# gmarcais/Jellyfish

Hardware: NVIDIA H100
Metric: k-mers counted/sec at k=21 (higher is better)
Workload: dtype u64

## Files before the change

jellyfish_b200/csrc/jf_device.cuh:

```cuda
#ifndef JF_DEVICE_CUH
#define JF_DEVICE_CUH
#include <stdint.h>
#include <cuda_runtime.h>
#include <type_traits>

namespace jfk {

constexpr int HALO  = 256;
constexpr int PRE   = 64;

enum { ST_H = 0, ST_S = 1, ST_L = 2 };
constexpr uint32_t SYM_BREAK = 4;

enum { STAT_KMERS = 0, STAT_INSERTED, STAT_DISTINCT, STAT_REPROBES, STAT_OVERFLOWED,
       STAT_FAILED, STAT_FAIL_DROPPED, STAT_OVF_FULL, STAT_ROUTE_DROPPED, STAT_MAXCOUNT, STAT_POOL_FULL, STAT_FORMAT_ERR, STAT_N };

struct Carry {
  uint32_t state;
  uint32_t pad;
  uint8_t  sym[PRE];
};

struct TableDev {
  void*     slots;
  uint64_t  local_mask;
  uint32_t  local_lsize;
  uint32_t  lsize;
  uint32_t  shard_index;
  uint32_t  kbits;
  uint32_t  rbits;
  uint32_t  fbits;
  uint32_t  max_reprobe;
  uint32_t  op;
  unsigned long long* ovf_keys;
  unsigned long long* ovf_vals;
  uint64_t  ovf_mask;
  unsigned long long* stats;
  uint64_t* fail_keys;
  uint64_t* fail_counts;
  uint64_t  fail_cap;
};

enum { BLOOM_NONE = 0, BLOOM_FILTER = 1, BLOOM_COUNT = 2, BLOOM_CHECK = 3 };
struct BloomDev {
  uint32_t mode;
  uint32_t k;
  uint64_t m;
  uint64_t inv;
  uint32_t* bits;
  uint32_t* locks;
  uint32_t lock_mask;
  uint32_t pad;
  const uint64_t* lut1;
  const uint64_t* lut2;
};

struct u128 { uint64_t lo, hi; };

__host__ __device__ __forceinline__ uint64_t tri(uint32_t i) { return (uint64_t)i * (i + 1) / 2; }

__device__ __forceinline__ uint32_t smem_u32(const void* p) { return (uint32_t)__cvta_generic_to_shared(p); }

__device__ __forceinline__ void mbar_init(uint64_t* bar, uint32_t count) {
  asm volatile("mbarrier.init.shared::cta.b64 [%0], %1;" :: "r"(smem_u32(bar)), "r"(count) : "memory");
}
__device__ __forceinline__ void mbar_expect_tx(uint64_t* bar, uint32_t bytes) {
  asm volatile("mbarrier.arrive.expect_tx.shared::cta.b64 _, [%0], %1;" :: "r"(smem_u32(bar)), "r"(bytes) : "memory");
}
__device__ __forceinline__ void mbar_arrive(uint64_t* bar) {
  asm volatile("mbarrier.arrive.shared::cta.b64 _, [%0];" :: "r"(smem_u32(bar)) : "memory");
}
__device__ __forceinline__ bool mbar_try_wait(uint64_t* bar, uint32_t parity) {
  uint32_t ok;
  asm volatile("{\n\t.reg .pred p;\n\t"
               "mbarrier.try_wait.parity.shared::cta.b64 p, [%1], %2;\n\t"
               "selp.u32 %0, 1, 0, p;\n\t}"
               : "=r"(ok) : "r"(smem_u32(bar)), "r"(parity) : "memory");
  return ok != 0;
}
__device__ __forceinline__ void mbar_wait(uint64_t* bar, uint32_t parity) {
  while(!mbar_try_wait(bar, parity)) { }
}
__device__ __forceinline__ void tma_load_1d(void* dst, const void* src, uint32_t bytes, uint64_t* bar) {
  asm volatile("cp.async.bulk.shared::cluster.global.mbarrier::complete_tx::bytes [%0], [%1], %2, [%3];"
               :: "r"(smem_u32(dst)), "l"(src), "r"(bytes), "r"(smem_u32(bar)) : "memory");
}
__device__ __forceinline__ void tma_store_1d(void* dst, const void* src, uint32_t bytes) {
  asm volatile("cp.async.bulk.global.shared::cta.bulk_group [%0], [%1], %2;" :: "l"(dst), "r"(smem_u32(src)), "r"(bytes) : "memory");
}
__device__ __forceinline__ void tma_commit_group() { asm volatile("cp.async.bulk.commit_group;" ::: "memory"); }
__device__ __forceinline__ void tma_wait_group_read0() { asm volatile("cp.async.bulk.wait_group.read 0;" ::: "memory"); }
__device__ __forceinline__ void tma_wait_group0() { asm volatile("cp.async.bulk.wait_group 0;" ::: "memory"); }
__device__ __forceinline__ void fence_proxy_async() {
  asm volatile("fence.proxy.async.shared::cta;" ::: "memory");
}

__device__ __forceinline__ u128 atomic_cas_128(void* addr, u128 cmp, u128 val) {
  u128 old;
  asm volatile("{\n\t.reg .b128 c, s, d;\n\t"
               "mov.b128 c, {%2, %3};\n\t"
               "mov.b128 s, {%4, %5};\n\t"
               "atom.global.relaxed.gpu.cas.b128 d, [%6], c, s;\n\t"
               "mov.b128 {%0, %1}, d;\n\t}"
               : "=l"(old.lo), "=l"(old.hi)
               : "l"(cmp.lo), "l"(cmp.hi), "l"(val.lo), "l"(val.hi), "l"(addr) : "memory");
  return old;
}
__device__ __forceinline__ u128 load_128(const void* addr) {
  u128 v;
  asm volatile("ld.global.relaxed.gpu.v2.u64 {%0, %1}, [%2];" : "=l"(v.lo), "=l"(v.hi) : "l"(addr) : "memory");
  return v;
}

__host__ __device__ __forceinline__ uint32_t base_symbol(uint32_t b) {
  uint32_t u = b & 0xDFu;
  uint32_t x = (b >> 1) & 3u;
  uint32_t code = x ^ (x >> 1);
  bool ok = (u == 'A') | (u == 'C') | (u == 'G') | (u == 'T');
  return ok ? code : SYM_BREAK;
}
// ... 349 lines not shown
```

jellyfish_b200/csrc/jf_engine.cu:

```cuda
#include <cuda_runtime.h>
#include <algorithm>
#include <atomic>
#include <cmath>
#include <cstdio>
#include <cstring>
#include <string>
#include <vector>

#include "../../include/jfgpu.h"
#include "host/jf_matrix.hpp"
#include "jf_kernels.cuh"
#include "jf_extract.cuh"
#include "jf_window.cuh"
#include "jf_dump.cuh"
#include "jf_shard.cuh"

using namespace jfk;

static std::atomic<unsigned long long> g_launches(0);
static thread_local std::string g_create_error;

#define JF_LAUNCHED() g_launches.fetch_add(1, std::memory_order_relaxed)

namespace {
// ... 1042 lines not shown
  TableDev T = table_dev(e, e->tab);
  const uint64_t ns = e->tab.local_size + e->tab.margin;
  const int grid = (int)std::min<uint64_t>((ns + 255) / 256, (uint64_t)e->n_sm * 16);
  switch(e->tab.slot_bits) {
  case 32:  max_count_kernel<32><<<grid, 256, 0, e->cs>>>(T, ns); break;
  case 64:  max_count_kernel<64><<<grid, 256, 0, e->cs>>>(T, ns); break;
  default:  max_count_kernel<128><<<grid, 256, 0, e->cs>>>(T, ns); break;
  }
  JF_LAUNCHED();
  int rc = read_stats(e);
  if(rc) return rc;
  const uint64_t maxc = e->h_stats[STAT_MAXCOUNT];
  if(e->eff_val_len < 64 && (maxc >> e->eff_val_len) != 0) {
    e->eff_val_len = bitsize(maxc);
    if(!e->tab.M.is_identity()) {
      rc = rebuild_table(e, e->tab.lsize, jfb::gf2_matrix::identity(kbits), 0, 0);
      if(rc) return rc;
    }
  }
  return JFGPU_OK;
}

void resolve_kernel_events(jfgpu_engine* e) {
  for(size_t i = 0; i + 1 < e->kev_used; i += 2) {
    float ms = 0;
    if(cudaEventElapsedTime(&ms, e->kev[i], e->kev[i + 1]) == cudaSuccess) { e->kernel_ms += ms; e->kernel_launches++; }
    else cudaGetLastError();
  }
  e->kev_used = 0;
}

int check_after_batches(jfgpu_engine* e) {
  int rc = read_stats(e);
  if(rc) return rc;
  if(e->h_stats[STAT_OVF_FULL]) return fail(e, JFGPU_ERR_FULL, "counter overflow side table is full");
  if(e->h_stats[STAT_FAILED]) {
    if(e->part.pending) {
      rc = part_drain(e, e->cs);
      if(rc) return rc;
      rc = read_stats(e);
      if(rc) return rc;
      if(!e->h_stats[STAT_FAILED]) return JFGPU_OK;
    }
    return regrow(e);
  }
  return JFGPU_OK;
}

}

extern "C" {

const char* jfgpu_version(void) { return "jellyfish-b200 0.1 (sm_90a)"; }
uint64_t jfgpu_kernel_launches(void) { return g_launches.load(); }
const char* jfgpu_last_error(jfgpu_handle h) { return h ? h->err.c_str() : g_create_error.c_str(); }

void* jfgpu_host_alloc(size_t bytes) { void* p = nullptr; if(cudaHostAlloc(&p, bytes, cudaHostAllocDefault) != cudaSuccess) { cudaGetLastError(); return nullptr; } return p; }
void jfgpu_host_free(void* p) { if(p) cudaFreeHost(p); }
int jfgpu_memcpy_h2d(void* dev_dst, const void* host_src, size_t bytes, void* stream) {
  if(cudaMemcpyAsync(dev_dst, host_src, bytes, cudaMemcpyHostToDevice, (cudaStream_t)stream) != cudaSuccess) { cudaGetLastError(); return JFGPU_ERR_CUDA; }
  return JFGPU_OK;
}

int jfgpu_reference_matrix(uint32_t r, uint32_t c, uint32_t skip, uint64_t* cols) {
  if(r == 0 || r > 64 || c == 0 || !cols) return JFGPU_ERR_ARG;
  jfb::glibc_random rng;
  jfb::gf2_matrix res;
  for(uint32_t i = 0; i <= skip; ++i) { jfb::gf2_matrix m(r, c); res = m.randomize_pseudo_inverse(rng); }
  for(uint32_t i = 0; i < c; ++i) cols[i] = res[i];
  return JFGPU_OK;
}

int jfgpu_create(const jfgpu_params* params, jfgpu_handle* out) {
  if(!params || !out) return fail(nullptr, JFGPU_ERR_ARG, "null argument");
  if(params->struct_size != sizeof(jfgpu_params)) return fail(nullptr, JFGPU_ERR_ARG, "jfgpu_params size mismatch");
  if(params->k < 1 || params->k > 64) return fail(nullptr, JFGPU_ERR_ARG, "mer length must be in [1, 64]");
  if(params->size == 0) return fail(nullptr, JFGPU_ERR_ARG, "size must be positive");
  uint32_t ns = params->n_shards ? params->n_shards : 1;
  if(ns & (ns - 1)) return fail(nullptr, JFGPU_ERR_ARG, "n_shards must be a power of two");
  if(params->shard_index >= ns) return fail(nullptr, JFGPU_ERR_ARG, "shard_index out of range");
  if(params->max_reprobe > 255) return fail(nullptr, JFGPU_ERR_ARG, "max_reprobe must be <= 255");

  int ndev = 0;
  if(cudaGetDeviceCount(&ndev) != cudaSuccess || ndev == 0) {
    cudaGetLastError();
    return fail(nullptr, JFGPU_ERR_CUDA, "no CUDA device: the jellyfish-b200 engine has no CPU fallback");
  }
  if(params->device < 0 || params->device >= ndev) return fail(nullptr, JFGPU_ERR_ARG, "invalid device ordinal");

  jfgpu_engine* e = new jfgpu_engine;
  e->p = *params;
  e->p.n_shards = ns;
  e->device = params->device;
  e->k = params->k;
  e->kw = params->k > 32 ? 2 : 1;
  e->nbytes = (2 * params->k + 7) / 8;
  e->eff_val_len = params->counter_len;
  e->shard_bits = ceil_log2(ns);
  auto bail = [&](int code) { g_create_error = e->err; jfgpu_destroy(e); return code; };

  cudaError_t c;
  if((c = cudaSetDevice(e->device)) != cudaSuccess) { e->err = cudaGetErrorString(c); return bail(JFGPU_ERR_CUDA); }
  cudaDeviceProp prop;
  if((c = cudaGetDeviceProperties(&prop, e->device)) != cudaSuccess) { e->err = cudaGetErrorString(c); return bail(JFGPU_ERR_CUDA); }
  if(prop.major != 9 || prop.minor != 0) { e->err = "this engine is built for sm_90a (Hopper) only"; return bail(JFGPU_ERR_CUDA); }
  e->n_sm = prop.multiProcessorCount;
  if(cudaStreamCreateWithFlags(&e->cs, cudaStreamNonBlocking) != cudaSuccess ||
// ... 739 lines not shown
```

jellyfish_b200/csrc/jf_window.cuh:

```cuda
#pragma once

namespace jfk {

constexpr uint32_t WIN_TILE_UNITS = 4;
constexpr uint32_t WIN_MAX_G = 64;
constexpr uint32_t WIN_MAX_WPR = 2048;
constexpr uint32_t WIN_NTH = 512;

struct WinDev {
  uint32_t g0, G, wpr_lg, n_tiles;
  const uint32_t* lazy_win;
  uint32_t tile_first[WIN_MAX_G + 1];
  uint32_t stile_first[WIN_MAX_G + 1];
  uint32_t unit_first[WIN_MAX_G + 1];
  uint32_t* wstart;
  uint32_t* wcursor;
  uint32_t* wcnt;
  uint32_t* wrec; uint64_t wrec_cap;
  uint64_t* def_pos; uint32_t* def_high; unsigned long long* def_n; uint64_t def_cap;
};

__device__ __forceinline__ uint32_t win_region_of_tile(const WinDev& wd, uint32_t tile) {
  uint32_t r = 0;
  while(r + 1 < wd.G && wd.tile_first[r + 1] <= tile) ++r;
  return r;
}

__device__ __forceinline__ uint64_t win_slot_base(const WinDev& wd, uint32_t region_bits, uint32_t task) {
  return ((uint64_t)(wd.g0 + (task >> wd.wpr_lg)) << region_bits) + ((uint64_t)(task & ((1u << wd.wpr_lg) - 1)) << WIN_LG);
}

__global__ void __launch_bounds__(WIN_NTH) win_hist_kernel(PartDev pd, WinDev wd, const uint32_t* __restrict__ order, uint32_t hb) {
  __shared__ uint32_t cnt[WIN_MAX_WPR];
  const uint32_t wpr = 1u << wd.wpr_lg;
  for(uint32_t i = threadIdx.x; i < wpr; i += WIN_NTH) cnt[i] = 0;
  __syncthreads();
  const uint32_t r = win_region_of_tile(wd, blockIdx.x);
  const uint32_t u0 = wd.unit_first[r] + (blockIdx.x - wd.tile_first[r]) * WIN_TILE_UNITS;
  const uint32_t u1 = min(u0 + WIN_TILE_UNITS, wd.unit_first[r + 1]);
  uint32_t chunk[WIN_TILE_UNITS], n[WIN_TILE_UNITS]; uint4 v[WIN_TILE_UNITS];
#pragma unroll
  for(uint32_t j = 0; j < WIN_TILE_UNITS; ++j) chunk[j] = u0 + j < u1 ? __ldg(order + u0 + j) : 0u;
#pragma unroll
  for(uint32_t j = 0; j < WIN_TILE_UNITS; ++j) n[j] = u0 + j < u1 ? __ldg(&pd.dir[chunk[j]].y) : 0u;
#pragma unroll
  for(uint32_t j = 0; j < WIN_TILE_UNITS; ++j) {
    v[j] = make_uint4(0, 0, 0, 0);
    if(threadIdx.x * 4 < n[j]) v[j] = __ldg(reinterpret_cast<const uint4*>(pd.pool + (size_t)chunk[j] * CHUNK_BYTES) + threadIdx.x);
  }
#pragma unroll
  for(uint32_t j = 0; j < WIN_TILE_UNITS; ++j) {
    const uint32_t i = threadIdx.x * 4;
    const uint32_t rec[4] = { v[j].x, v[j].y, v[j].z, v[j].w };
// ... 56 lines not shown
  const uint32_t half = tid >> 9, piece = tid & 511u;
  const uint32_t wmask = wpr - 1;
#pragma unroll
  for(uint32_t it = 0; it < WIN_ST_UNITS / 2; ++it) {
    const uint32_t j = 2 * it + half, n = s_n[j];
    if(piece * 4 < n) {
      const uint4 v = __ldg(reinterpret_cast<const uint4*>(pd.pool + (size_t)s_chunk[j] * CHUNK_BYTES) + piece);
      const uint32_t rec[4] = { v.x, v.y, v.z, v.w };
#pragma unroll
      for(uint32_t q = 0; q < 4; ++q) if(piece * 4 + q < n) atomicAdd(&cnt[((rec[q] >> hb) >> WIN_LG) & wmask], 1u);
    }
  }
  __syncthreads();
  const uint32_t per = (wpr + WIN_ST_NTH - 1) / WIN_ST_NTH;
  const uint32_t b = tid * per;
  uint32_t s = 0;
  for(uint32_t i = b; i < min(b + per, wpr); ++i) s += cnt[i];
  uint32_t incl = s;
#pragma unroll
  for(int o = 1; o < 32; o <<= 1) { const uint32_t v = __shfl_up_sync(0xffffffffu, incl, o); if((tid & 31) >= (uint32_t)o) incl += v; }
  if((tid & 31) == 31) warp_tot[tid >> 5] = incl;
  __syncthreads();
  uint32_t woff = 0, total = 0;
  for(uint32_t w = 0; w < WIN_ST_NTH / 32; ++w) { const uint32_t x = warp_tot[w]; if(w < (tid >> 5)) woff += x; total += x; }
  uint32_t run = woff + incl - s;
  for(uint32_t i = b; i < min(b + per, wpr); ++i) {
    const uint32_t c = cnt[i];
    lbase[i] = run; lcur[i] = run;
    gbase[i] = (c ? atomicAdd(&wd.wcursor[(r << wd.wpr_lg) + i], c) : 0u) - run;
    run += c;
  }
  __syncthreads();
#pragma unroll
  for(uint32_t it = 0; it < WIN_ST_UNITS / 2; ++it) {
    const uint32_t j = 2 * it + half, n = s_n[j];
    if(piece * 4 < n) {
      const uint4 v = __ldcs(reinterpret_cast<const uint4*>(pd.pool + (size_t)s_chunk[j] * CHUNK_BYTES) + piece);
      const uint32_t rec[4] = { v.x, v.y, v.z, v.w };
#pragma unroll
      for(uint32_t q = 0; q < 4; ++q) if(piece * 4 + q < n) stage[atomicAdd(&lcur[((rec[q] >> hb) >> WIN_LG) & wmask], 1u)] = rec[q];
    }
  }
  __syncthreads();
  for(uint32_t i = tid; i < total; i += WIN_ST_NTH) {
    const uint32_t v = stage[i], w = ((v >> hb) >> WIN_LG) & wmask;
    const uint32_t dst = gbase[w] + i;
    if(dst < wd.wrec_cap) wd.wrec[dst] = v;
  }
}

constexpr uint32_t WIN2_NTH = 1024;
constexpr uint32_t WIN2_CONS = WIN2_NTH - 32;
constexpr uint32_t WIN2_RB  = 10240;
constexpr uint32_t WIN2_BLK = 256;
constexpr uint32_t WIN2_NONE = 0xFFFFFFFFu;
constexpr size_t   WIN2_SMEM = (size_t)2 * WIN_SLOTS * 4 + (size_t)2 * WIN2_RB * 4;

struct Win2Info { uint32_t task, b, n, pad; };

template<int KW>
__global__ void __launch_bounds__(WIN2_NTH, 1) win_insert2_kernel(TableDev T, PartDev pd, WinDev wd, const uint64_t* __restrict__ inv_lut_g, uint32_t nbytes) {
  extern __shared__ __align__(128) uint8_t w2smem[];
  __shared__ __align__(8) uint64_t full[2];
  __shared__ __align__(8) uint64_t empty[2];
  __shared__ Win2Info info[2];
  __shared__ uint32_t cursor[2];
  uint32_t* const winb0 = reinterpret_cast<uint32_t*>(w2smem);
  uint32_t* const recb0 = winb0 + 2 * WIN_SLOTS;
  uint32_t* tab = (uint32_t*)T.slots;
  const uint32_t n_tasks = wd.G << wd.wpr_lg;
  const uint32_t tid = threadIdx.x, lane = tid & 31u;

  auto slot_base_of = [&](uint32_t task) -> uint64_t { return win_slot_base(wd, pd.region_bits, task); };
  if(tid == 0) {
    mbar_init(&full[0], 1); mbar_init(&full[1], 1);
    mbar_init(&empty[0], WIN2_CONS / 32); mbar_init(&empty[1], WIN2_CONS / 32);
    fence_proxy_async();
  }
  __syncthreads();

  if(tid < 32) {
    const bool lead = lane == 0;
    uint32_t next_from = blockIdx.x;
    uint32_t ephase[2] = { 0, 0 };
    uint32_t cur_task[2] = { WIN2_NONE, WIN2_NONE }, cur_n[2] = { 0, 0 }, cur_b[2] = { 0, 0 };
    auto load_batch = [&](uint32_t s, uint32_t off, bool with_window) {
      const uint32_t nb = min(WIN2_RB, cur_n[s] - off);
      const uint32_t rbytes = ((nb + 3u) & ~3u) * 4u;
      cursor[s] = 0;
      mbar_expect_tx(&full[s], rbytes + (with_window ? WIN_SLOTS * 4u : 0u));
      if(with_window) tma_load_1d(winb0 + s * WIN_SLOTS, tab + slot_base_of(cur_task[s]), WIN_SLOTS * 4u, &full[s]);
      tma_load_1d(recb0 + s * WIN2_RB, wd.wrec + cur_b[s] + off, rbytes, &full[s]);
    };
    auto next_window = [&](uint32_t s) {
      uint32_t t = next_from, c = 0;
      while(t < n_tasks && (c = wd.wcnt[t]) == 0) t += gridDim.x;
      if(t >= n_tasks) {
        next_from = t; cur_task[s] = WIN2_NONE;
        if(lead) { info[s].task = WIN2_NONE; mbar_arrive(&full[s]); }
        return;
      }
      next_from = t + gridDim.x;
      cur_task[s] = t; cur_n[s] = c; cur_b[s] = wd.wstart[t];
      const bool fill = wd.lazy_win && wd.lazy_win[slot_base_of(t) >> WIN_LG] != WIN_IN_MEMORY;
      if(fill) {
        uint4* const w = reinterpret_cast<uint4*>(winb0 + s * WIN_SLOTS);
        for(uint32_t i = lane; i < WIN_SLOTS / 4; i += 32) w[i] = make_uint4(0, 0, 0, 0);
        fence_proxy_async();
        __syncwarp();
      }
      if(lead) {
        info[s].task = t; info[s].b = cur_b[s]; info[s].n = c;
        load_batch(s, 0, !fill);
      }
    };
    next_window(0); next_window(1);
    for(uint32_t s = 0; cur_task[s] != WIN2_NONE; s ^= 1u) {
      for(uint32_t off = WIN2_RB; off < cur_n[s]; off += WIN2_RB) {
        mbar_wait(&empty[s], ephase[s]); ephase[s] ^= 1u;
        if(lead) load_batch(s, off, false);
      }
      mbar_wait(&empty[s], ephase[s]); ephase[s] ^= 1u;
      if(lead) {
        tma_store_1d(tab + slot_base_of(cur_task[s]), winb0 + s * WIN_SLOTS, WIN_SLOTS * 4u);
        tma_commit_group();
        tma_wait_group_read0();
      }
      __syncwarp();
      next_window(s);
    }
    if(lead) tma_wait_group0();
    return;
  }

  const uint32_t fb = T.fbits, rb = T.rbits, hb = fb - rb;
  const uint32_t fmask = (1u << fb) - 1u, one = 1u << fb, cb = 32 - fb;
  const uint32_t hmask = hb ? ((1u << hb) - 1u) : 0u;
  const uint32_t lt_mask = (1u << lane) - 1u;
  uint32_t n_ins = 0, n_new = 0, n_rep = 0;
  uint32_t fphase[2] = { 0, 0 };
  for(uint32_t s = 0; ; s ^= 1u) {
    mbar_wait(&full[s], fphase[s]); fphase[s] ^= 1u;
    const Win2Info inf = info[s];
    if(inf.task == WIN2_NONE) break;
    uint32_t* const win = winb0 + s * WIN_SLOTS;
    const uint32_t* const recs = recb0 + s * WIN2_RB;
    const uint64_t slot_base = slot_base_of(inf.task);
    for(uint32_t off = 0; off < inf.n; off += WIN2_RB) {
      const uint32_t nb = min(WIN2_RB, inf.n - off);
      if(off) { mbar_wait(&full[s], fphase[s]); fphase[s] ^= 1u; }
      bool have = false, want = true;
      uint32_t rec = 0, local = 0, kf = 0, at = 0, p = 0;
      uint32_t blk_next = 0, blk_end = 0;
      bool more = true;
      for(;;) {
        const uint32_t need = __ballot_sync(0xffffffffu, want);
        if(need && more) {
          if(blk_next >= blk_end) {
            uint32_t base = 0;
            if(lane == 0) base = atomicAdd(&cursor[s], WIN2_BLK);
            blk_next = __shfl_sync(0xffffffffu, base, 0);
            blk_end = min(blk_next + WIN2_BLK, nb);
            more = blk_next < nb;
          }
          if(want && more) {
            const uint32_t i = blk_next + __popc(need & lt_mask);
            if(i < blk_end) {
              rec = recs[i];
              local = (rec >> hb) & (WIN_SLOTS - 1); kf = ((rec & hmask) << rb) | 1u;
              at = local; p = 0;
              have = true; want = false;
            }
          }
          blk_next = min(blk_next + (uint32_t)__popc(need), blk_end);
        }
        if(!__any_sync(0xffffffffu, have)) { if(!more) break; else continue; }
        if(have) {
          if(at < WIN_SLOTS) {
            const uint32_t o = atomicCAS(&win[at], 0u, kf | one);
            if(o == 0u) { ++n_new; ++n_ins; n_rep += p; want = true; }
            else if((o & fmask) == kf) {
              const uint32_t o2 = atomicAdd(&win[at], one);
              if((((o2 >> fb) + 1) >> cb) != 0) k2_carry(T.ovf_keys, T.ovf_vals, T.ovf_mask, T.stats, slot_base + at);
              ++n_ins; n_rep += p; want = true;
            } else if(p < T.max_reprobe) { ++p; at += p; ++kf; }
            else {
              k2_fail<KW>(T.shard_index, T.local_lsize, T.lsize, T.stats, T.fail_keys, T.fail_counts, T.fail_cap, slot_base + local, rec & hmask, inv_lut_g, nbytes);
              want = true;
            }
          } else {
            const unsigned long long d = atomicAdd(wd.def_n, 1ull);
            if(d < wd.def_cap) { wd.def_pos[d] = slot_base + local; wd.def_high[d] = rec & hmask; }
            else atomicAdd(&T.stats[STAT_POOL_FULL], 1ull);
            want = true;
          }
          have = !want;
        }
      }
      fence_proxy_async();
      __syncwarp();
      if(lane == 0) mbar_arrive(&empty[s]);
    }
  }
  unsigned long long v[3] = { n_ins, n_new, n_rep };
#pragma unroll
  for(int q = 0; q < 3; ++q) {
#pragma unroll
    for(int o = 16; o; o >>= 1) v[q] += __shfl_xor_sync(0xffffffffu, v[q], o);
  }
  if(lane == 0) {
    if(v[0]) atomicAdd(&T.stats[STAT_INSERTED], v[0]);
    if(v[1]) atomicAdd(&T.stats[STAT_DISTINCT], v[1]);
    if(v[2]) atomicAdd(&T.stats[STAT_REPROBES], v[2]);
  }
}

__global__ void __launch_bounds__(256) win_zero_kernel(uint32_t* __restrict__ tab, const uint32_t* __restrict__ state, const uint32_t* __restrict__ wcnt,
                                                       uint64_t w_first, uint32_t n) {
  const uint32_t lane = threadIdx.x & 31u;
  const uint32_t n_warps = gridDim.x * (blockDim.x / 32);
  for(uint32_t t = (blockIdx.x * blockDim.x + threadIdx.x) / 32; t < n; t += n_warps) {
    if((wcnt && wcnt[t]) || state[w_first + t] == WIN_IN_MEMORY) continue;
    uint4* const w = reinterpret_cast<uint4*>(tab + ((w_first + t) << WIN_LG));
    for(uint32_t i = lane; i < WIN_SLOTS / 4; i += 32) w[i] = make_uint4(0, 0, 0, 0);
  }
}

template<int KW>
__global__ void __launch_bounds__(256) win_deferred_kernel(TableDev T, WinDev wd, const uint64_t* __restrict__ inv_lut_g, uint32_t nbytes) {
  const uint32_t fb = T.fbits, rb = T.rbits;
  const uint32_t fmask = (1u << fb) - 1u, one = 1u << fb, cb = 32 - fb;
  uint32_t* tab = (uint32_t*)T.slots;
  const unsigned long long n = min(*wd.def_n, (unsigned long long)wd.def_cap);
  uint32_t n_ins = 0, n_new = 0, n_rep = 0;
  for(unsigned long long i = (unsigned long long)blockIdx.x * blockDim.x + threadIdx.x; i < n; i += (unsigned long long)gridDim.x * blockDim.x) {
    const uint64_t base = wd.def_pos[i];
    const uint32_t high = wd.def_high[i], kf0 = high << rb;
    bool ok = true;
    const uint32_t o = atomicCAS(&tab[base], 0u, (kf0 | 1u) | one);
    if(o == 0u) ++n_new;
    else if((o & fmask) == (kf0 | 1u)) {
      const uint32_t o2 = atomicAdd(&tab[base], one);
      if((((o2 >> fb) + 1) >> cb) != 0) k2_carry(T.ovf_keys, T.ovf_vals, T.ovf_mask, T.stats, base);
    } else {
      const uint32_t w = k2_walk(tab, base, kf0, fb, T.max_reprobe);
      ok = w != 0;
      if(ok) {
        const uint32_t p = (w & 0xFFFFu) - 1;
        n_rep += p; if(w & 0x10000u) ++n_new;
        if(w & 0x20000u) k2_carry(T.ovf_keys, T.ovf_vals, T.ovf_mask, T.stats, base + tri(p));
      }
    }
    if(ok) ++n_ins;
    else k2_fail<KW>(T.shard_index, T.local_lsize, T.lsize, T.stats, T.fail_keys, T.fail_counts, T.fail_cap, base, high, inv_lut_g, nbytes);
  }
  unsigned long long v[3] = { n_ins, n_new, n_rep };
// ... 14 lines not shown
```

Before: 36.20 billion.

## Restructure window insert pipeline: batched metadata lookup, early record prefetch, two-phase probing

The producer warp now scans window metadata 32 tasks at a time with a ballot, and issues the next window's record TMA load before waiting on the store of the current window, so the loads overlap the write-back. Consumer warps now do a vectorized first-probe pass over 64-record blocks, two records per lane. Records that collide go into a per-warp shared-memory queue and are reprobed in a second phase, which keeps lanes busy and lets the kernel use smaller blocks. It also adds optional clock64 instrumentation behind a compile flag. The changes add extra shared memory and a more complex mbarrier expect_tx protocol, which makes correctness harder to verify.

```diff
diff --git a/jellyfish_b200/csrc/jf_device.cuh b/jellyfish_b200/csrc/jf_device.cuh
--- a/jellyfish_b200/csrc/jf_device.cuh
+++ b/jellyfish_b200/csrc/jf_device.cuh
@@ -66,6 +66,9 @@
 }
 __device__ __forceinline__ void mbar_expect_tx(uint64_t* bar, uint32_t bytes) {
   asm volatile("mbarrier.arrive.expect_tx.shared::cta.b64 _, [%0], %1;" :: "r"(smem_u32(bar)), "r"(bytes) : "memory");
+}
+__device__ __forceinline__ void mbar_expect_tx_only(uint64_t* bar, uint32_t bytes) {
+  asm volatile("mbarrier.expect_tx.relaxed.cta.shared::cta.b64 [%0], %1;" :: "r"(smem_u32(bar)), "r"(bytes) : "memory");
 }
 __device__ __forceinline__ void mbar_arrive(uint64_t* bar) {
   asm volatile("mbarrier.arrive.shared::cta.b64 _, [%0];" :: "r"(smem_u32(bar)) : "memory");
diff --git a/jellyfish_b200/csrc/jf_engine.cu b/jellyfish_b200/csrc/jf_engine.cu
--- a/jellyfish_b200/csrc/jf_engine.cu
+++ b/jellyfish_b200/csrc/jf_engine.cu
@@ -1118,6 +1118,15 @@
 extern "C" {
 
 const char* jfgpu_version(void) { return "jellyfish-b200 0.1 (sm_90a)"; }
+
+#ifdef JF_K2C_CLOCKS
+int jfgpu_k2c_clocks(uint64_t* out) {
+  unsigned long long z[jfk::K2C_N] = {};
+  if(cudaDeviceSynchronize() != cudaSuccess || cudaMemcpyFromSymbol(out, jfk::k2c_clocks, sizeof(z)) != cudaSuccess ||
+     cudaMemcpyToSymbol(jfk::k2c_clocks, z, sizeof(z)) != cudaSuccess) return JFGPU_ERR_CUDA;
+  return JFGPU_OK;
+}
+#endif
 uint64_t jfgpu_kernel_launches(void) { return g_launches.load(); }
 const char* jfgpu_last_error(jfgpu_handle h) { return h ? h->err.c_str() : g_create_error.c_str(); }
 
diff --git a/jellyfish_b200/csrc/jf_window.cuh b/jellyfish_b200/csrc/jf_window.cuh
--- a/jellyfish_b200/csrc/jf_window.cuh
+++ b/jellyfish_b200/csrc/jf_window.cuh
@@ -161,11 +161,21 @@
 constexpr uint32_t WIN2_NTH = 1024;
 constexpr uint32_t WIN2_CONS = WIN2_NTH - 32;
 constexpr uint32_t WIN2_RB  = 10240;
-constexpr uint32_t WIN2_BLK = 256;
+constexpr uint32_t WIN2_BLK = 64;
+constexpr uint32_t WIN2_QCAP = 96;
 constexpr uint32_t WIN2_NONE = 0xFFFFFFFFu;
-constexpr size_t   WIN2_SMEM = (size_t)2 * WIN_SLOTS * 4 + (size_t)2 * WIN2_RB * 4;
+constexpr size_t   WIN2_SMEM = (size_t)2 * WIN_SLOTS * 4 + (size_t)2 * WIN2_RB * 4 + (size_t)(WIN2_CONS / 32) * WIN2_QCAP * 4;
 
 struct Win2Info { uint32_t task, b, n, pad; };
+
+enum { K2C_P_EMPTY, K2C_P_STORE, K2C_P_META, K2C_P_ZERO, K2C_P_REC, K2C_P_TOTAL, K2C_WINDOWS, K2C_BATCHES,
+       K2C_C_FULL, K2C_C_PROBE, K2C_C_TRIPS, K2C_C_PROBES, K2C_C_TOTAL, K2C_N };
+#ifdef JF_K2C_CLOCKS
+__device__ unsigned long long k2c_clocks[K2C_N];
+#define K2C(x) x
+#else
+#define K2C(x)
+#endif
 
 template<int KW>
 __global__ void __launch_bounds__(WIN2_NTH, 1) win_insert2_kernel(TableDev T, PartDev pd, WinDev wd, const uint64_t* __restrict__ inv_lut_g, uint32_t nbytes) {
@@ -174,6 +184,7 @@
   __shared__ __align__(8) uint64_t empty[2];
   __shared__ Win2Info info[2];
   __shared__ uint32_t cursor[2];
+  K2C(__shared__ long long ck_issue[2];)
   uint32_t* const winb0 = reinterpret_cast<uint32_t*>(w2smem);
   uint32_t* const recb0 = winb0 + 2 * WIN_SLOTS;
   uint32_t* tab = (uint32_t*)T.slots;
@@ -190,55 +201,98 @@
 
   if(tid < 32) {
     const bool lead = lane == 0;
-    uint32_t next_from = blockIdx.x;
-    uint32_t ephase[2] = { 0, 0 };
-    uint32_t cur_task[2] = { WIN2_NONE, WIN2_NONE }, cur_n[2] = { 0, 0 }, cur_b[2] = { 0, 0 };
-    auto load_batch = [&](uint32_t s, uint32_t off, bool with_window) {
-      const uint32_t nb = min(WIN2_RB, cur_n[s] - off);
-      const uint32_t rbytes = ((nb + 3u) & ~3u) * 4u;
-      cursor[s] = 0;
-      mbar_expect_tx(&full[s], rbytes + (with_window ? WIN_SLOTS * 4u : 0u));
-      if(with_window) tma_load_1d(winb0 + s * WIN_SLOTS, tab + slot_base_of(cur_task[s]), WIN_SLOTS * 4u, &full[s]);
-      tma_load_1d(recb0 + s * WIN2_RB, wd.wrec + cur_b[s] + off, rbytes, &full[s]);
-    };
-    auto next_window = [&](uint32_t s) {
-      uint32_t t = next_from, c = 0;
-      while(t < n_tasks && (c = wd.wcnt[t]) == 0) t += gridDim.x;
-      if(t >= n_tasks) {
-        next_from = t; cur_task[s] = WIN2_NONE;
-        if(lead) { info[s].task = WIN2_NONE; mbar_arrive(&full[s]); }
-        return;
-      }
-      next_from = t + gridDim.x;
-      cur_task[s] = t; cur_n[s] = c; cur_b[s] = wd.wstart[t];
-      const bool fill = wd.lazy_win && wd.lazy_win[slot_base_of(t) >> WIN_LG] != WIN_IN_MEMORY;
-      if(fill) {
+    uint32_t look_from = blockIdx.x, look_base = 0;
+    uint32_t l_cnt = 0, l_b = 0, l_fill = 0, l_mask = 0;
+    K2C(unsigned long long ck[K2C_N] = {}; const long long ck_t0 = clock64(); long long ck_t;)
+    auto lookup = [&]() {
+      K2C(const long long t0 = clock64();)
+      while(l_mask == 0 && look_from < n_tasks) {
+        const uint32_t t = look_from + lane * gridDim.x;
+        const bool in = t < n_tasks;
+        l_cnt = in ? wd.wcnt[t] : 0u;
+        l_b = in ? wd.wstart[t] : 0u;
+        l_fill = in && wd.lazy_win && wd.lazy_win[slot_base_of(t) >> WIN_LG] != WIN_IN_MEMORY;
+        l_mask = __ballot_sync(0xffffffffu, l_cnt != 0);
+        look_base = look_from; look_from += 32u * gridDim.x;
+      }
+      K2C(ck[K2C_P_META] += clock64() - t0;)
+    };
+    struct Stage { uint32_t task, n, b, fill, ephase; };
+    auto next_window = [&](Stage& S) {
+      if(l_mask == 0) lookup();
+      if(l_mask == 0) { S.task = WIN2_NONE; return; }
+      const uint32_t j = __ffs(l_mask) - 1; l_mask &= l_mask - 1;
+      S.task = look_base + j * gridDim.x;
+      S.n = __shfl_sync(0xffffffffu, l_cnt, j); S.b = __shfl_sync(0xffffffffu, l_b, j); S.fill = __shfl_sync(0xffffffffu, l_fill, j);
+    };
+    auto load_records = [&](uint32_t s, const Stage& S, uint32_t off, bool arrive) {
+      K2C(ck_issue[s] = clock64(); ++ck[K2C_BATCHES];)
+      const uint32_t rbytes = ((min(WIN2_RB, S.n - off) + 3u) & ~3u) * 4u;
+      if(arrive) { cursor[s] = 0; mbar_expect_tx(&full[s], rbytes); }
+      else mbar_expect_tx_only(&full[s], rbytes);
+      tma_load_1d(recb0 + s * WIN2_RB, wd.wrec + S.b + off, rbytes, &full[s]);
+    };
+    auto start_window = [&](uint32_t s, const Stage& S) {
+      K2C(++ck[K2C_WINDOWS];)
+      if(S.fill) {
+        K2C(const long long t0 = clock64();)
         uint4* const w = reinterpret_cast<uint4*>(winb0 + s * WIN_SLOTS);
         for(uint32_t i = lane; i < WIN_SLOTS / 4; i += 32) w[i] = make_uint4(0, 0, 0, 0);
         fence_proxy_async();
         __syncwarp();
+        K2C(ck[K2C_P_ZERO] += clock64() - t0;)
       }
       if(lead) {
-        info[s].task = t; info[s].b = cur_b[s]; info[s].n = c;
-        load_batch(s, 0, !fill);
-      }
-    };
-    next_window(0); next_window(1);
-    for(uint32_t s = 0; cur_task[s] != WIN2_NONE; s ^= 1u) {
-      for(uint32_t off = WIN2_RB; off < cur_n[s]; off += WIN2_RB) {
-        mbar_wait(&empty[s], ephase[s]); ephase[s] ^= 1u;
-        if(lead) load_batch(s, off, false);
-      }
-      mbar_wait(&empty[s], ephase[s]); ephase[s] ^= 1u;
+        info[s].task = S.task; info[s].b = S.b; info[s].n = S.n;
+        cursor[s] = 0;
+        if(S.fill) mbar_arrive(&full[s]);
+        else {
+          mbar_expect_tx(&full[s], WIN_SLOTS * 4u);
+          tma_load_1d(winb0 + s * WIN_SLOTS, tab + slot_base_of(S.task), WIN_SLOTS * 4u, &full[s]);
+        }
+      }
+    };
+    auto first_window = [&](uint32_t s, Stage& S) {
+      S.ephase = 0;
+      next_window(S);
+      if(S.task == WIN2_NONE) { if(lead) { info[s].task = WIN2_NONE; mbar_arrive(&full[s]); } return; }
+      if(lead) load_records(s, S, 0, false);
+      start_window(s, S);
+    };
+    auto serve = [&](uint32_t s, Stage& S) {
+      for(uint32_t off = WIN2_RB; off < S.n; off += WIN2_RB) {
+        K2C(ck_t = clock64();)
+        mbar_wait(&empty[s], S.ephase); S.ephase ^= 1u;
+        K2C(ck[K2C_P_EMPTY] += clock64() - ck_t;)
+        if(lead) load_records(s, S, off, true);
+      }
+      Stage N; N.ephase = S.ephase ^ 1u;
+      next_window(N);
+      K2C(ck_t = clock64();)
+      mbar_wait(&empty[s], S.ephase);
+      K2C({ const long long n = clock64(); ck[K2C_P_EMPTY] += n - ck_t; ck_t = n; })
       if(lead) {
-        tma_store_1d(tab + slot_base_of(cur_task[s]), winb0 + s * WIN_SLOTS, WIN_SLOTS * 4u);
+        tma_store_1d(tab + slot_base_of(S.task), winb0 + s * WIN_SLOTS, WIN_SLOTS * 4u);
         tma_commit_group();
+        if(N.task != WIN2_NONE) load_records(s, N, 0, false);
         tma_wait_group_read0();
       }
       __syncwarp();
-      next_window(s);
+      K2C(ck[K2C_P_STORE] += clock64() - ck_t;)
+      if(N.task == WIN2_NONE) { if(lead) { info[s].task = WIN2_NONE; mbar_arrive(&full[s]); } }
+      else start_window(s, N);
+      S = N;
+      if(l_mask == 0) lookup();
+    };
+    Stage S0, S1;
+    first_window(0, S0); first_window(1, S1);
+    while(S0.task != WIN2_NONE) {
+      serve(0, S0);
+      if(S1.task == WIN2_NONE) break;
+      serve(1, S1);
     }
     if(lead) tma_wait_group0();
+    K2C(if(lead) { ck[K2C_P_TOTAL] = clock64() - ck_t0; for(int q = 0; q < K2C_C_FULL; ++q) atomicAdd(&k2c_clocks[q], ck[q]); })
     return;
   }
 
@@ -246,71 +300,106 @@
   const uint32_t fmask = (1u << fb) - 1u, one = 1u << fb, cb = 32 - fb;
   const uint32_t hmask = hb ? ((1u << hb) - 1u) : 0u;
   const uint32_t lt_mask = (1u << lane) - 1u;
+  uint32_t* const wq = recb0 + 2 * WIN2_RB + (tid / 32 - 1) * WIN2_QCAP;
   uint32_t n_ins = 0, n_new = 0, n_rep = 0;
-  uint32_t fphase[2] = { 0, 0 };
+  uint32_t fphase = 0;
+  K2C(unsigned long long ck[K2C_N] = {}; const long long ck_t0 = clock64(); long long ck_t;)
   for(uint32_t s = 0; ; s ^= 1u) {
-    mbar_wait(&full[s], fphase[s]); fphase[s] ^= 1u;
+    K2C(ck_t = clock64();)
+    mbar_wait(&full[s], (fphase >> s) & 1u); fphase ^= 1u << s;
+    K2C({ const long long n = clock64(); ck[K2C_C_FULL] += n - ck_t; ck_t = n; })
     const Win2Info inf = info[s];
     if(inf.task == WIN2_NONE) break;
+    K2C(if(tid == 32) ck[K2C_P_REC] += ck_t - ck_issue[s];)
     uint32_t* const win = winb0 + s * WIN_SLOTS;
     const uint32_t* const recs = recb0 + s * WIN2_RB;
     const uint64_t slot_base = slot_base_of(inf.task);
     for(uint32_t off = 0; off < inf.n; off += WIN2_RB) {
       const uint32_t nb = min(WIN2_RB, inf.n - off);
-      if(off) { mbar_wait(&full[s], fphase[s]); fphase[s] ^= 1u; }
-      bool have = false, want = true;
+      K2C(ck_t = clock64();)
+      if(off) { mbar_wait(&full[s], (fphase >> s) & 1u); fphase ^= 1u << s; }
+      K2C({ const long long n = clock64(); ck[K2C_C_FULL] += n - ck_t; ck_t = n; if(off && tid == 32) ck[K2C_P_REC] += n - ck_issue[s]; })
+      uint32_t qn = 0;
+      bool more = true;
+      bool have = false;
       uint32_t rec = 0, local = 0, kf = 0, at = 0, p = 0;
-      uint32_t blk_next = 0, blk_end = 0;
-      bool more = true;
       for(;;) {
-        const uint32_t need = __ballot_sync(0xffffffffu, want);
-        if(need && more) {
-          if(blk_next >= blk_end) {
-            uint32_t base = 0;
-            if(lane == 0) base = atomicAdd(&cursor[s], WIN2_BLK);
-            blk_next = __shfl_sync(0xffffffffu, base, 0);
-            blk_end = min(blk_next + WIN2_BLK, nb);
-            more = blk_next < nb;
+        uint32_t base = 0;
+        if(lane == 0) base = atomicAdd(&cursor[s], WIN2_BLK);
+        base = __shfl_sync(0xffffffffu, base, 0);
+        more = base < nb;
+        if(more) {
+          const uint32_t i0 = base + lane * 2;
+          uint2 r2 = make_uint2(0, 0);
+          if(i0 < nb) r2 = *reinterpret_cast<const uint2*>(recs + i0);
+          const uint32_t r[2] = { r2.x, r2.y };
+          uint32_t o[2] = { 0, 0 };
+#pragma unroll
+          for(uint32_t q = 0; q < 2; ++q)
+            if(i0 + q < nb) o[q] = atomicCAS(&win[(r[q] >> hb) & (WIN_SLOTS - 1)], 0u, (((r[q] & hmask) << rb) | 1u) | one);
+          K2C(++ck[K2C_C_TRIPS]; ck[K2C_C_PROBES] += __reduce_add_sync(0xffffffffu, i0 < nb ? min(2u, nb - i0) : 0u);)
+#pragma unroll
+          for(uint32_t q = 0; q < 2; ++q) {
+            bool queue = false;
+            if(i0 + q < nb) {
+              const uint32_t l = (r[q] >> hb) & (WIN_SLOTS - 1), k = ((r[q] & hmask) << rb) | 1u;
+              if(o[q] == 0u) { ++n_new; ++n_ins; }
+              else if((o[q] & fmask) == k) {
+                const uint32_t o2 = atomicAdd(&win[l], one);
+                if((((o2 >> fb) + 1) >> cb) != 0) k2_carry(T.ovf_keys, T.ovf_vals, T.ovf_mask, T.stats, slot_base + l);
+                ++n_ins;
+              } else queue = true;
+            }
+            const uint32_t bq = __ballot_sync(0xffffffffu, queue);
+            if(queue) wq[qn + __popc(bq & lt_mask)] = r[q];
+            qn += __popc(bq);
           }
-          if(want && more) {
-            const uint32_t i = blk_next + __popc(need & lt_mask);
-            if(i < blk_end) {
-              rec = recs[i];
-              local = (rec >> hb) & (WIN_SLOTS - 1); kf = ((rec & hmask) << rb) | 1u;
-              at = local; p = 0;
-              have = true; want = false;
+          __syncwarp();
+        }
+        for(;;) {
+          const uint32_t idle = __ballot_sync(0xffffffffu, !have);
+          const uint32_t n_idle = __popc(idle);
+          if(more ? qn < n_idle : (qn == 0 && n_idle == 32)) break;
+          if(!have) {
+            const uint32_t k = __popc(idle & lt_mask);
+            if(k < qn) {
+              rec = wq[qn - 1 - k];
+              local = (rec >> hb) & (WIN_SLOTS - 1); kf = ((rec & hmask) << rb) | 1u; at = local; p = 0;
+              have = true;
             }
           }
-          blk_next = min(blk_next + (uint32_t)__popc(need), blk_end);
-        }
-        if(!__any_sync(0xffffffffu, have)) { if(!more) break; else continue; }
-        if(have) {
-          if(at < WIN_SLOTS) {
-            const uint32_t o = atomicCAS(&win[at], 0u, kf | one);
-            if(o == 0u) { ++n_new; ++n_ins; n_rep += p; want = true; }
-            else if((o & fmask) == kf) {
-              const uint32_t o2 = atomicAdd(&win[at], one);
-              if((((o2 >> fb) + 1) >> cb) != 0) k2_carry(T.ovf_keys, T.ovf_vals, T.ovf_mask, T.stats, slot_base + at);
-              ++n_ins; n_rep += p; want = true;
-            } else if(p < T.max_reprobe) { ++p; at += p; ++kf; }
-            else {
-              k2_fail<KW>(T.shard_index, T.local_lsize, T.lsize, T.stats, T.fail_keys, T.fail_counts, T.fail_cap, slot_base + local, rec & hmask, inv_lut_g, nbytes);
-              want = true;
-            }
-          } else {
+          qn -= min(qn, n_idle);
+          __syncwarp();
+          K2C(++ck[K2C_C_TRIPS]; ck[K2C_C_PROBES] += __popc(__ballot_sync(0xffffffffu, have));)
+          if(!have) continue;
+          if(p >= T.max_reprobe) {
+            k2_fail<KW>(T.shard_index, T.local_lsize, T.lsize, T.stats, T.fail_keys, T.fail_counts, T.fail_cap, slot_base + local, rec & hmask, inv_lut_g, nbytes);
+            have = false; continue;
+          }
+          ++p; at += p; ++kf;
+          if(at >= WIN_SLOTS) {
             const unsigned long long d = atomicAdd(wd.def_n, 1ull);
             if(d < wd.def_cap) { wd.def_pos[d] = slot_base + local; wd.def_high[d] = rec & hmask; }
             else atomicAdd(&T.stats[STAT_POOL_FULL], 1ull);
-            want = true;
+            have = false; continue;
           }
-          have = !want;
+          const uint32_t o1 = atomicCAS(&win[at], 0u, kf | one);
+          if(o1 == 0u) { ++n_new; ++n_ins; n_rep += p; have = false; }
+          else if((o1 & fmask) == kf) {
+            const uint32_t o2 = atomicAdd(&win[at], one);
+            if((((o2 >> fb) + 1) >> cb) != 0) k2_carry(T.ovf_keys, T.ovf_vals, T.ovf_mask, T.stats, slot_base + at);
+            ++n_ins; n_rep += p; have = false;
+          }
         }
-      }
+        if(!more) break;
+      }
+      K2C(ck[K2C_C_PROBE] += clock64() - ck_t;)
       fence_proxy_async();
       __syncwarp();
       if(lane == 0) mbar_arrive(&empty[s]);
     }
   }
+  K2C(if(lane == 0) { ck[K2C_C_TOTAL] = clock64() - ck_t0; for(int q = K2C_C_FULL; q < K2C_N; ++q) atomicAdd(&k2c_clocks[q], ck[q]); if(tid == 32) atomicAdd(&k2c_clocks[K2C_P_REC], ck[K2C_P_REC]); })
   unsigned long long v[3] = { n_ins, n_new, n_rep };
 #pragma unroll
   for(int q = 0; q < 3; ++q) {
```

Result: faster. 36.67 billion (median of 6 runs) (+1.3%).

## Add batched first-probe sweep to window insert with survivor compaction

Applied to the files above, without the earlier changes.

Consumer warps now take a 256-record block, issue the first-probe CAS for all records in unrolled sweeps, and handle hits and own-key increments inline. Only records whose first slot held a different key are compacted back into shared memory and go through the per-lane reprobe loop, which starts at probe 1. The producer loop is specialized per stage with compile-time stage indices, and optional clock64 instrumentation is added behind a compile flag. This is meant to cut the ballot/shuffle overhead per record in the common first-probe case, at the cost of extra shared-memory rewrites and more complex control flow.

```diff
diff --git a/jellyfish_b200/csrc/jf_engine.cu b/jellyfish_b200/csrc/jf_engine.cu
--- a/jellyfish_b200/csrc/jf_engine.cu
+++ b/jellyfish_b200/csrc/jf_engine.cu
@@ -1119,6 +1119,14 @@
 
 const char* jfgpu_version(void) { return "jellyfish-b200 0.1 (sm_90a)"; }
 uint64_t jfgpu_kernel_launches(void) { return g_launches.load(); }
+#ifdef JF_K2C_CLOCKS
+int jfgpu_k2c_clocks(uint64_t* out) {
+  const size_t bytes = sizeof(unsigned long long) * K2C_MAX_CTAS * K2C_N;
+  if(cudaDeviceSynchronize() != cudaSuccess || cudaMemcpyFromSymbol(out, g_k2c_clocks, bytes) != cudaSuccess) return JFGPU_ERR_CUDA;
+  std::vector<unsigned long long> zero(K2C_MAX_CTAS * K2C_N, 0ull);
+  return cudaMemcpyToSymbol(g_k2c_clocks, zero.data(), bytes) == cudaSuccess ? JFGPU_OK : JFGPU_ERR_CUDA;
+}
+#endif
 const char* jfgpu_last_error(jfgpu_handle h) { return h ? h->err.c_str() : g_create_error.c_str(); }
 
 void* jfgpu_host_alloc(size_t bytes) { void* p = nullptr; if(cudaHostAlloc(&p, bytes, cudaHostAllocDefault) != cudaSuccess) { cudaGetLastError(); return nullptr; } return p; }
diff --git a/jellyfish_b200/csrc/jf_window.cuh b/jellyfish_b200/csrc/jf_window.cuh
--- a/jellyfish_b200/csrc/jf_window.cuh
+++ b/jellyfish_b200/csrc/jf_window.cuh
@@ -1,4 +1,6 @@
 #pragma once
+
+#include <type_traits>
 
 namespace jfk {
 
@@ -167,6 +169,31 @@
 
 struct Win2Info { uint32_t task, b, n, pad; };
 
+enum { K2C_CONS_FULL, K2C_CONS_PROBE, K2C_CONS_ALL, K2C_PROD_EMPTY, K2C_PROD_ALL, K2C_N };
+constexpr uint32_t K2C_MAX_CTAS = 1024;
+#ifdef JF_K2C_CLOCKS
+__device__ unsigned long long g_k2c_clocks[K2C_MAX_CTAS * K2C_N];
+struct K2cClocks {
+  unsigned long long c[2];
+  long long t0, t;
+  __device__ __forceinline__ K2cClocks() { c[0] = c[1] = 0; t = t0 = clock64(); }
+  __device__ __forceinline__ void mark() { t = clock64(); }
+  __device__ __forceinline__ void add(int q) { c[q] += clock64() - t; }
+  __device__ __forceinline__ void flush(uint32_t first, uint32_t n) {
+    if((threadIdx.x & 31u) || blockIdx.x >= K2C_MAX_CTAS) return;
+    unsigned long long* const g = g_k2c_clocks + blockIdx.x * K2C_N + first;
+    for(uint32_t q = 0; q < n; ++q) atomicAdd(g + q, c[q]);
+    atomicAdd(g + n, (unsigned long long)(clock64() - t0));
+  }
+};
+#else
+struct K2cClocks {
+  __device__ __forceinline__ void mark() {}
+  __device__ __forceinline__ void add(int) {}
+  __device__ __forceinline__ void flush(uint32_t, uint32_t) {}
+};
+#endif
+
 template<int KW>
 __global__ void __launch_bounds__(WIN2_NTH, 1) win_insert2_kernel(TableDev T, PartDev pd, WinDev wd, const uint64_t* __restrict__ inv_lut_g, uint32_t nbytes) {
   extern __shared__ __align__(128) uint8_t w2smem[];
@@ -191,9 +218,10 @@
   if(tid < 32) {
     const bool lead = lane == 0;
     uint32_t next_from = blockIdx.x;
-    uint32_t ephase[2] = { 0, 0 };
+    uint32_t ephase = 0;
     uint32_t cur_task[2] = { WIN2_NONE, WIN2_NONE }, cur_n[2] = { 0, 0 }, cur_b[2] = { 0, 0 };
-    auto load_batch = [&](uint32_t s, uint32_t off, bool with_window) {
+    auto load_batch = [&](auto S, uint32_t off, bool with_window) {
+      constexpr uint32_t s = decltype(S)::value;
       const uint32_t nb = min(WIN2_RB, cur_n[s] - off);
       const uint32_t rbytes = ((nb + 3u) & ~3u) * 4u;
       cursor[s] = 0;
@@ -201,7 +229,8 @@
       if(with_window) tma_load_1d(winb0 + s * WIN_SLOTS, tab + slot_base_of(cur_task[s]), WIN_SLOTS * 4u, &full[s]);
       tma_load_1d(recb0 + s * WIN2_RB, wd.wrec + cur_b[s] + off, rbytes, &full[s]);
     };
-    auto next_window = [&](uint32_t s) {
+    auto next_window = [&](auto S) {
+      constexpr uint32_t s = decltype(S)::value;
       uint32_t t = next_from, c = 0;
       while(t < n_tasks && (c = wd.wcnt[t]) == 0) t += gridDim.x;
       if(t >= n_tasks) {
@@ -220,25 +249,33 @@
       }
       if(lead) {
         info[s].task = t; info[s].b = cur_b[s]; info[s].n = c;
-        load_batch(s, 0, !fill);
+        load_batch(S, 0, !fill);
       }
     };
-    next_window(0); next_window(1);
-    for(uint32_t s = 0; cur_task[s] != WIN2_NONE; s ^= 1u) {
+    K2cClocks clk;
+    auto run_stage = [&](auto S) -> bool {
+      constexpr uint32_t s = decltype(S)::value;
+      if(cur_task[s] == WIN2_NONE) return false;
       for(uint32_t off = WIN2_RB; off < cur_n[s]; off += WIN2_RB) {
-        mbar_wait(&empty[s], ephase[s]); ephase[s] ^= 1u;
-        if(lead) load_batch(s, off, false);
-      }
-      mbar_wait(&empty[s], ephase[s]); ephase[s] ^= 1u;
+        clk.mark(); mbar_wait(&empty[s], (ephase >> s) & 1u); ephase ^= 1u << s; clk.add(0);
+        if(lead) load_batch(S, off, false);
+      }
+      clk.mark(); mbar_wait(&empty[s], (ephase >> s) & 1u); ephase ^= 1u << s; clk.add(0);
       if(lead) {
         tma_store_1d(tab + slot_base_of(cur_task[s]), winb0 + s * WIN_SLOTS, WIN_SLOTS * 4u);
         tma_commit_group();
         tma_wait_group_read0();
       }
       __syncwarp();
-      next_window(s);
-    }
+      next_window(S);
+      return true;
+    };
+    const std::integral_constant<uint32_t, 0> stage_0;
+    const std::integral_constant<uint32_t, 1> stage_1;
+    next_window(stage_0); next_window(stage_1);
+    while(run_stage(stage_0) && run_stage(stage_1)) { }
     if(lead) tma_wait_group0();
+    clk.flush(K2C_PROD_EMPTY, 1);
     return;
   }
 
@@ -246,71 +283,121 @@
   const uint32_t fmask = (1u << fb) - 1u, one = 1u << fb, cb = 32 - fb;
   const uint32_t hmask = hb ? ((1u << hb) - 1u) : 0u;
   const uint32_t lt_mask = (1u << lane) - 1u;
+  constexpr uint32_t SWEEP = WIN2_BLK / 32;
   uint32_t n_ins = 0, n_new = 0, n_rep = 0;
-  uint32_t fphase[2] = { 0, 0 };
+  uint32_t fphase = 0;
+  K2cClocks clk;
   for(uint32_t s = 0; ; s ^= 1u) {
-    mbar_wait(&full[s], fphase[s]); fphase[s] ^= 1u;
+    clk.mark(); mbar_wait(&full[s], (fphase >> s) & 1u); fphase ^= 1u << s; clk.add(K2C_CONS_FULL);
     const Win2Info inf = info[s];
     if(inf.task == WIN2_NONE) break;
     uint32_t* const win = winb0 + s * WIN_SLOTS;
-    const uint32_t* const recs = recb0 + s * WIN2_RB;
+    uint32_t* const recs = recb0 + s * WIN2_RB;
     const uint64_t slot_base = slot_base_of(inf.task);
     for(uint32_t off = 0; off < inf.n; off += WIN2_RB) {
       const uint32_t nb = min(WIN2_RB, inf.n - off);
-      if(off) { mbar_wait(&full[s], fphase[s]); fphase[s] ^= 1u; }
-      bool have = false, want = true;
+      if(off) { clk.mark(); mbar_wait(&full[s], (fphase >> s) & 1u); fphase ^= 1u << s; clk.add(K2C_CONS_FULL); }
+      clk.mark();
+      bool have = false;
       uint32_t rec = 0, local = 0, kf = 0, at = 0, p = 0;
-      uint32_t blk_next = 0, blk_end = 0;
+      uint32_t sv_next = 0, sv_end = 0;
       bool more = true;
       for(;;) {
-        const uint32_t need = __ballot_sync(0xffffffffu, want);
-        if(need && more) {
-          if(blk_next >= blk_end) {
-            uint32_t base = 0;
-            if(lane == 0) base = atomicAdd(&cursor[s], WIN2_BLK);
-            blk_next = __shfl_sync(0xffffffffu, base, 0);
-            blk_end = min(blk_next + WIN2_BLK, nb);
-            more = blk_next < nb;
+        const uint32_t need = __ballot_sync(0xffffffffu, !have);
+        if(need && sv_next == sv_end && more) {
+          uint32_t base = 0;
+          if(lane == 0) base = atomicAdd(&cursor[s], WIN2_BLK);
+          base = __shfl_sync(0xffffffffu, base, 0);
+          more = base < nb;
+          if(more) {
+            const uint32_t cnt = min(WIN2_BLK, nb - base);
+            uint32_t r[SWEEP], o[SWEEP];
+#pragma unroll
+            for(uint32_t u = 0; u < SWEEP; ++u) r[u] = u * 32 + lane < cnt ? recs[base + u * 32 + lane] : 0u;
+#pragma unroll
+            for(uint32_t u = 0; u < SWEEP; ++u) {
+              o[u] = 0u;
+              if(u * 32 + lane < cnt) o[u] = atomicCAS(&win[(r[u] >> hb) & (WIN_SLOTS - 1)], 0u, (((r[u] & hmask) << rb) | 1u) | one);
+            }
+            uint32_t sv_bits = 0, rare_bits = 0;
+#pragma unroll
+            for(uint32_t u = 0; u < SWEEP; ++u) {
+              const bool valid = u * 32 + lane < cnt;
+              const bool own = o[u] != 0u && (o[u] & fmask) == (((r[u] & hmask) << rb) | 1u);
+              n_new += valid && o[u] == 0u;
+              n_ins += valid && (o[u] == 0u || own);
+              sv_bits |= (uint32_t)(valid && o[u] != 0u && !own) << u;
+              if(own) {
+                const uint32_t o2 = atomicAdd(&win[(r[u] >> hb) & (WIN_SLOTS - 1)], one);
+                rare_bits |= (uint32_t)((((o2 >> fb) + 1) >> cb) != 0) << u;
+              }
+            }
+            if(!T.max_reprobe) { rare_bits |= sv_bits; sv_bits = 0; }
+            if(__any_sync(0xffffffffu, rare_bits)) {
+#pragma unroll 1
+              for(uint32_t u = 0; u < SWEEP; ++u) {
+                if(!((rare_bits >> u) & 1u)) continue;
+                const uint32_t x = recs[base + u * 32 + lane], l = (x >> hb) & (WIN_SLOTS - 1);
+                if((win[l] & fmask) == (((x & hmask) << rb) | 1u)) k2_carry(T.ovf_keys, T.ovf_vals, T.ovf_mask, T.stats, slot_base + l);
+                else k2_fail<KW>(T.shard_index, T.local_lsize, T.lsize, T.stats, T.fail_keys, T.fail_counts, T.fail_cap, slot_base + l, x & hmask, inv_lut_g, nbytes);
+              }
+            }
+#pragma unroll
+            for(uint32_t u = 0; u < SWEEP; ++u) r[u] = (sv_bits >> u) & 1u ? recs[base + u * 32 + lane] : 0u;
+            const uint32_t c = __popc(sv_bits);
+            uint32_t incl = c;
+#pragma unroll
+            for(int d = 1; d < 32; d <<= 1) { const uint32_t t = __shfl_up_sync(0xffffffffu, incl, d); if(lane >= (uint32_t)d) incl += t; }
+            const uint32_t n_sv = __shfl_sync(0xffffffffu, incl, 31);
+            __syncwarp();
+            uint32_t* dst = recs + base + incl - c;
+#pragma unroll
+            for(uint32_t u = 0; u < SWEEP; ++u) if((sv_bits >> u) & 1u) *dst++ = r[u];
+            __syncwarp();
+            sv_next = base; sv_end = base + n_sv;
           }
-          if(want && more) {
-            const uint32_t i = blk_next + __popc(need & lt_mask);
-            if(i < blk_end) {
+        }
+        if(need && sv_next < sv_end) {
+          if(!have) {
+            const uint32_t i = sv_next + __popc(need & lt_mask);
+            if(i < sv_end) {
               rec = recs[i];
-              local = (rec >> hb) & (WIN_SLOTS - 1); kf = ((rec & hmask) << rb) | 1u;
-              at = local; p = 0;
-              have = true; want = false;
+              local = (rec >> hb) & (WIN_SLOTS - 1); kf = (((rec & hmask) << rb) | 1u) + 1u;
+              at = local + 1; p = 1;
+              have = true;
             }
           }
-          blk_next = min(blk_next + (uint32_t)__popc(need), blk_end);
+          sv_next = min(sv_next + (uint32_t)__popc(need), sv_end);
         }
-        if(!__any_sync(0xffffffffu, have)) { if(!more) break; else continue; }
+        if(!__any_sync(0xffffffffu, have)) { if(!more && sv_next == sv_end) break; else continue; }
         if(have) {
           if(at < WIN_SLOTS) {
             const uint32_t o = atomicCAS(&win[at], 0u, kf | one);
-            if(o == 0u) { ++n_new; ++n_ins; n_rep += p; want = true; }
+            if(o == 0u) { ++n_new; ++n_ins; n_rep += p; have = false; }
             else if((o & fmask) == kf) {
               const uint32_t o2 = atomicAdd(&win[at], one);
               if((((o2 >> fb) + 1) >> cb) != 0) k2_carry(T.ovf_keys, T.ovf_vals, T.ovf_mask, T.stats, slot_base + at);
-              ++n_ins; n_rep += p; want = true;
+              ++n_ins; n_rep += p; have = false;
             } else if(p < T.max_reprobe) { ++p; at += p; ++kf; }
             else {
               k2_fail<KW>(T.shard_index, T.local_lsize, T.lsize, T.stats, T.fail_keys, T.fail_counts, T.fail_cap, slot_base + local, rec & hmask, inv_lut_g, nbytes);
-              want = true;
+              have = false;
             }
           } else {
             const unsigned long long d = atomicAdd(wd.def_n, 1ull);
             if(d < wd.def_cap) { wd.def_pos[d] = slot_base + local; wd.def_high[d] = rec & hmask; }
             else atomicAdd(&T.stats[STAT_POOL_FULL], 1ull);
-            want = true;
+            have = false;
           }
-          have = !want;
         }
       }
       fence_proxy_async();
       __syncwarp();
+      clk.add(K2C_CONS_PROBE);
       if(lane == 0) mbar_arrive(&empty[s]);
     }
   }
+  clk.flush(K2C_CONS_FULL, 2);
   unsigned long long v[3] = { n_ins, n_new, n_rep };
 #pragma unroll
   for(int q = 0; q < 3; ++q) {
```

Result: faster. 35.88 billion before, 36.95 billion after (median of 6 runs) (+3.0%).
